# ParthaEth/GIF

Hardware: AMD Instinct MI355X
Metric: G+D train-step images/sec at 256x256, batch 32/GPU (higher is better)
Workload: dtype f32

## Files before the change

gif_amd/csrc/conv_igemm.hip:

```cpp
#include <stdlib.h>

#include <atomic>
#include <type_traits>

#include "conv_common.h"
#include "conv_route.h"

namespace {

using gif::f32x16, gif::f32x4, gif::xcd_remap;
using gif::buf_rsrc_t, gif::make_buf_rsrc, gif::buf_load_lds16;

struct GatherParams {
    const void* x;
    const void* wp;
    void* y;
    const float* in_scale;
    const float* out_scale;
    const float* bias;
    const void* residual;
    int B, Hi, Wi, Ci;
    int Ho, Wo, Co;
    int Hp, Wp;
    int os, ooy, oox;
// ... 822 lines not shown
#pragma unroll
        for (int j = 0; j < NT; ++j) bv[slot][j] = *reinterpret_cast<const frag_t*>(Bb + j * 32 * LD + c);
        if (SCALE) {
#pragma unroll
            for (int i = 0; i < MT; ++i)
                av[slot][i] *= *reinterpret_cast<const frag_t*>(Stab + s_row[i] + (pair ? (kk * 2 * EPC) & (BK / 2 - 1) : kc + kk * 2 * EPC));
        }
    };
    auto mfma_group = [&](int slot) __attribute__((always_inline)) {
        if constexpr (F16) {
#pragma unroll
            for (int i = 0; i < MT; ++i)
#pragma unroll
                for (int j = 0; j < NT; ++j)
                    acc[i][j] = __builtin_amdgcn_mfma_f32_32x32x16_f16(av[slot][i], bv[slot][j], acc[i][j], 0, 0, 0);
            __builtin_amdgcn_sched_group_barrier(0x100, MT + NT + (SCALE ? MT : 0), 0);
            __builtin_amdgcn_sched_group_barrier(0x008, MT * NT, 0);
        } else {
#pragma unroll
            for (int t = 0; t < 4; ++t)
#pragma unroll
                for (int i = 0; i < MT; ++i)
#pragma unroll
                    for (int j = 0; j < NT; ++j)
                        acc[i][j] = __builtin_amdgcn_mfma_f32_32x32x2f32(av[slot][i][t], bv[slot][j][t], acc[i][j], 0, 0, 0);
            __builtin_amdgcn_sched_group_barrier(0x100, MT + NT + (SCALE ? MT : 0), 0);
            __builtin_amdgcn_sched_group_barrier(0x008, 4 * MT * NT, 0);
        }
    };

    issue(0);
    __syncthreads();
    frag_read(0, 0, 0, 0);
    for (int step = 0; step + 1 < nsteps; ++step) {
        issue(cur ^ 1);
#pragma unroll
        for (int g = 0; g + 1 < KG; ++g) {
            frag_read(cur, g + 1, (g + 1) & 1, cmp_kc);
            mfma_group(g & 1);
        }
        __syncthreads();
        cmp_kc = next_kc(cmp_kc);
        cur ^= 1;
        frag_read(cur, 0, KG & 1, cmp_kc);
        mfma_group((KG - 1) & 1);
        if (KG & 1) {
#pragma unroll
            for (int i = 0; i < MT; ++i) av[0][i] = av[1][i];
#pragma unroll
            for (int j = 0; j < NT; ++j) bv[0][j] = bv[1][j];
        }
    }
#pragma unroll
    for (int g = 0; g < KG; ++g) {
        if (g + 1 < KG) frag_read(cur, g + 1, (g + 1) & 1, cmp_kc);
        mfma_group(g & 1);
    }
    }
    conv_epilogue<BM, BN, 32, MT, NT, T, THREADS>(p, acc, smem, m0, n0, wm0, wn0, tid, li, lh, HWp);
}

template <typename T, int BM, int BN, int WAVES_M, int WAVES_N, bool SCALE, int BK, int X3 = 0, int NST = 2>
__global__ void __launch_bounds__(64 * WAVES_M * WAVES_N, (X3 == 2 && WAVES_M * WAVES_N == 4) ? 2 : 1) conv_gather_mfma_glds(const GatherParams p) {
    glds_body<T, BM, BN, WAVES_M, WAVES_N, SCALE, BK, X3, NST>(p, (int)blockIdx.x, (int)gridDim.x);
}

struct MultiParams {
    GatherParams ph[4];
    int wg_end[4];
    int nph;
};

template <typename T, int BM, int BN, int WAVES_M, int WAVES_N, bool SCALE, int BK, int X3 = 0, int NST = 2>
__global__ void __launch_bounds__(64 * WAVES_M * WAVES_N, (X3 == 2 && WAVES_M * WAVES_N == 4) ? 2 : 1) conv_gather_mfma_glds_multi(const MultiParams mp) {
    const int b = (int)blockIdx.x;
    int k = 0;
    while (k + 1 < mp.nph && b >= mp.wg_end[k]) ++k;
    const int begin = k ? mp.wg_end[k - 1] : 0;
    glds_body<T, BM, BN, WAVES_M, WAVES_N, SCALE, BK, X3, NST>(mp.ph[k], b - begin, mp.wg_end[k] - begin);
}

constexpr int kRowsThinA = 288;

__global__ void __launch_bounds__(256, 2) conv3x3_rows_thin_h2(const GatherParams p) {
    constexpr int BM = 256, BN = 32, LD = 32, THREADS = 256, MT = 2, NT = 1, AROWS = kRowsThinA, A_IT = AROWS / 32;
    extern __shared__ __attribute__((aligned(16))) float smem[];
    float* const As = smem;
    typedef __attribute__((address_space(3))) void* lptr_t;
    const float* const px = static_cast<const float*>(p.x);
    const unsigned short* const pw = static_cast<const unsigned short*>(p.wp);

    const int tid = threadIdx.x, lane = tid & 63;
    const int wave = __builtin_amdgcn_readfirstlane(tid >> 6);
    const int li = lane & 31, lh = lane >> 5;
    const int wm0 = wave * 64;
    const int tile = xcd_remap((int)blockIdx.x, (int)gridDim.x);
    const int m0 = tile * BM;
    const int HWp = p.Hp * p.Wp;
    const int segw = p.Wp >= BM ? BM : p.Wp, seg = segw + 2, nseg = BM / segw;

    unsigned a_voff[A_IT], a_mask[A_IT];
#pragma unroll
    for (int it = 0; it < A_IT; ++it) {
        const int r = (tid >> 3) + 32 * it;
        const int sg = r / seg, j = r - sg * seg;
        const int ms = m0 + sg * segw;
        const bool in_tile = sg < nseg && ms < p.M;
        const int mm = in_tile ? ms : 0;
        const int b = mm / HWp, rr = mm - b * HWp;
        const int oy = rr / p.Wp, ox0 = rr - oy * p.Wp;
        const int ix = ox0 + j - 1;
        const bool okx = in_tile && (unsigned)ix < (unsigned)p.Wi;
        const int c4 = ((tid & 7) ^ ((r >> 1) & 7)) * 4;
        a_voff[it] = (unsigned)(((b * p.Hi + oy) * p.Wi + ix) * p.Ci + c4) * 4u;
        unsigned mk = 0;
#pragma unroll
        for (int d = 0; d < 3; ++d) mk |= ((okx && (unsigned)(oy + d - 1) < (unsigned)p.Hi) ? 1u : 0u) << d;
        a_mask[it] = mk;
    }
    const buf_rsrc_t rs_a = make_buf_rsrc(px - (size_t)p.Wi * p.Ci, 0xFFFFFFFFu);

    const int kch = p.CP / 32, nst = 3 * kch;
    auto issue_a = [&](int buf, int st) __attribute__((always_inline)) {
        const int ta = st / kch, kc = (st - ta * kch) * 32;
        const int dy = p.dy0 + ta * p.ddy;
        const int so = ((dy + 1) * p.Wi * p.Ci + kc) * 4;
        float* Ad = As + buf * AROWS * LD + wave * 8 * LD;
#pragma unroll
        for (int it = 0; it < A_IT; ++it) {
            const int r = (tid >> 3) + 32 * it;
            const int c4 = ((tid & 7) ^ ((r >> 1) & 7)) * 4;
            const unsigned bad = (__builtin_amdgcn_ubfe(a_mask[it], (unsigned)(dy + 1), 1u) - 1u) | ((kc + c4 < p.Ci) ? 0u : 0xFFFFFFFFu);
            buf_load_lds16(rs_a, (lptr_t)(Ad + it * 32 * LD), a_voff[it] | bad, so);
        }
    };
    gif::u32x4_t sb[2][3][2][2];
    auto issue_b = [&](auto set_tag, int st) __attribute__((always_inline)) {
        constexpr int set = decltype(set_tag)::value;
        const int ta = st / kch, kc = (st - ta * kch) * 32;
#pragma unroll
        for (int tb = 0; tb < 3; ++tb) {
            const int widx = (p.ky0 + ta * p.kstep) * p.KW + p.kx0 + tb * p.kstep;
#pragma unroll
            for (int q = 0; q < 2; ++q)
#pragma unroll
                for (int t = 0; t < 2; ++t)
                    sb[set][tb][q][t] = *reinterpret_cast<const gif::u32x4_t*>(pw + ((size_t)(widx * 2 + t) * p.RP + li) * p.CP + kc + q * 16 + lh * 8);
        }
    };

    f32x16 acc[MT][NT];
#pragma unroll
    for (int i = 0; i < MT; ++i)
#pragma unroll
        for (int r = 0; r < 16; ++r) acc[i][0][r] = 0.f;
    gif::H2Row hr[MT];
    int a_row[MT];
#pragma unroll
    for (int i = 0; i < MT; ++i) a_row[i] = wm0 + i * 32 + li + 2 * ((wm0 + i * 32) / segw);

    auto compute = [&](int buf, auto set_tag) __attribute__((always_inline)) {
        constexpr int set = decltype(set_tag)::value;
        const float* Ab = As + buf * AROWS * LD;
#pragma unroll
        for (int tb = 0; tb < 3; ++tb) {
            const int shift = p.dx0 + tb * p.ddx + 1;
#pragma unroll
            for (int q = 0; q < 2; ++q) {
                f32x4 ra[MT][2];
#pragma unroll
                for (int i = 0; i < MT; ++i) {
                    const int brow = a_row[i] + shift;
                    const int f = (brow >> 1) & 7;
#pragma unroll
                    for (int u = 0; u < 2; ++u) ra[i][u] = *reinterpret_cast<const f32x4*>(Ab + brow * LD + (((q * 4 + lh * 2 + u) ^ f) << 2));
                }
                gif::u32x4_t sa[2][MT];
                bool need = false;
#pragma unroll
                for (int i = 0; i < MT; ++i) gif::h2_observe(hr[i], gif::h2_group_max(ra[i][0], ra[i][1]), need);
                if (need) {
#pragma unroll
                    for (int i = 0; i < MT; ++i)
                        gif::h2_for_rows(lh, hr[i].dl, [&](int r, int d) __attribute__((always_inline)) { acc[i][0][r] = ldexpf(acc[i][0][r], d); });
                }
#pragma unroll
                for (int i = 0; i < MT; ++i)
#pragma unroll
                    for (int e = 0; e < 4; ++e) {
                        unsigned h, l;
                        gif::split_pair_h2(ra[i][e / 2][(e % 2) * 2], ra[i][e / 2][(e % 2) * 2 + 1], hr[i].sc, h, l);
                        sa[0][i][e] = h; sa[1][i][e] = l;
                    }
#pragma unroll
                for (int t3 = 0; t3 < 3; ++t3) {
                    const gif::X3Terms tm = gif::x3_terms<true>(t3);
#pragma unroll
                    for (int i = 0; i < MT; ++i)
                        acc[i][0] = __builtin_amdgcn_mfma_f32_32x32x16_f16(__builtin_bit_cast(gif::f16x8_t, sa[tm.a][i]),
                                                                           __builtin_bit_cast(gif::f16x8_t, sb[set][tb][q][tm.b]), acc[i][0], 0, 0, 0);
                }
            }
        }
    };

    issue_a(0, 0);
    issue_b(std::integral_constant<int, 0>{}, 0);
    __builtin_amdgcn_s_waitcnt(0x0F70);
    __syncthreads();
    for (int st = 0; st < nst; st += 2) {
        if (st + 1 < nst) {
            issue_a(1, st + 1);
            issue_b(std::integral_constant<int, 1>{}, st + 1);
        }
        compute(0, std::integral_constant<int, 0>{});
        __builtin_amdgcn_s_waitcnt(0x0F70);
        __syncthreads();
        if (st + 1 < nst) {
            if (st + 2 < nst) {
                issue_a(0, st + 2);
                issue_b(std::integral_constant<int, 0>{}, st + 2);
            }
            compute(1, std::integral_constant<int, 1>{});
            __builtin_amdgcn_s_waitcnt(0x0F70);
            __syncthreads();
        }
    }

    {
        bool wide = false;
#pragma unroll
        for (int i = 0; i < MT; ++i) wide |= gif::h2_wide(hr[i]);
        if (p.gate) {
            const bool wflag = p.wexp[p.RP + li] != 0;
            if (__builtin_amdgcn_ballot_w64(wide) != 0 && __builtin_amdgcn_ballot_w64(wflag) != 0 && lane == 0) atomicMax(p.gate, p.gate_gen);
        }
        const int wex = p.wexp[li];
#pragma unroll
        for (int i = 0; i < MT; ++i)
            gif::h2_for_rows(lh, hr[i].ex, [&](int r, int er) __attribute__((always_inline)) { acc[i][0][r] = ldexpf(acc[i][0][r], -(er + wex)); });
    }
    conv_epilogue<BM, BN, LD, MT, NT, float, THREADS, false, 2 * AROWS * LD>(p, acc, smem, m0, 0, wm0, 0, tid, li, lh, HWp);
}

template <int BN, int CP>
constexpr int halo_lds_floats() { return CP == 32 ? 5376 : 10496; }

template <int BN, int CP>
__global__ void __launch_bounds__(256, 3) conv_halo_f16(const GatherParams p) {
    typedef gif::f16 T;
    constexpr int TH = 16, TW = 16, BM = TH * TW;
    constexpr int CPP = CP / 8;
    constexpr int CPP_SHIFT = CPP == 4 ? 2 : 3;
    constexpr int PPS_SHIFT = CPP == 4 ? 2 : 1;
    constexpr int SWM = CPP - 1;
    constexpr int KG = CP / 16, MT = 2, NT = BN / 32;
    constexpr int HALO_HALFS = halo_lds_floats<BN, CP>() * 2;
    static_assert((CP == 32 || CP == 64) && (BN == 32 || BN == 64), "halo kernel configurations");
    extern __shared__ __attribute__((aligned(16))) float smem[];
    T* const Xs = reinterpret_cast<T*>(smem);
    T* const Wsm = Xs + HALO_HALFS;
    const T* const px = static_cast<const T*>(p.x);
    const T* const pw = static_cast<const T*>(p.wp);
    const T* const pzero = static_cast<const T*>(p.zero);
    typedef const __attribute__((address_space(1))) void* gptr_t;
    typedef __attribute__((address_space(3))) void* lptr_t;

    const int tid = threadIdx.x, lane = tid & 63;
    const int wave = __builtin_amdgcn_readfirstlane(tid >> 6);
    const int li = lane & 31, lh = lane >> 5;
    const int tile = xcd_remap((int)blockIdx.x, (int)gridDim.x);
    const int tpi = p.t2_tx * p.t2_ty;
    const int b = tile / tpi, tr = tile - b * tpi;
    const int tyi = tr / p.t2_tx, txi = tr - tyi * p.t2_tx;
    const int dy_min = p.ddy > 0 ? p.dy0 : p.dy0 + (p.nky - 1) * p.ddy;
    const int dx_min = p.ddx > 0 ? p.dx0 : p.dx0 + (p.nkx - 1) * p.ddx;
    const int HWh = TW + p.nkx - 1;
    const int nchunks = (TH + p.nky - 1) * HWh * CPP;
    const bool has_scale = p.in_scale != nullptr;

    {
        constexpr int QSTEP = 256 / CPP;
        const int dqy = QSTEP / HWh, dqx = QSTEP - dqy * HWh;
        int q = (wave * 64 + lane) >> CPP_SHIFT;
        int hy = q / HWh, hx = q - hy * HWh;
        const int cphys = lane & SWM;
        const T* const xb = px + (size_t)b * p.Hi * p.Wi * p.Ci;
        const int gy0 = tyi * TH + dy_min, gx0 = txi * TW + dx_min;
        for (int e0 = wave * 64; e0 < nchunks; e0 += 256) {
            const int c = cphys ^ ((q >> PPS_SHIFT) & SWM);
            const int gy = gy0 + hy, gx = gx0 + hx;
            const bool ok = e0 + lane < nchunks && (unsigned)gy < (unsigned)p.Hi && (unsigned)gx < (unsigned)p.Wi && c * 8 < p.Ci;
            const T* g = ok ? xb + ((gy * p.Wi + gx) * p.Ci + c * 8) : pzero;
            __builtin_amdgcn_global_load_lds((gptr_t)g, (lptr_t)(Xs + e0 * 8), 16, 0, 0);
            q += QSTEP;
            hx += dqx; hy += dqy;
            if (hx >= HWh) { hx -= HWh; ++hy; }
        }
    }
    {
        constexpr int WPT = BN * CPP;
        const int cphys = lane & SWM;
        if constexpr (WPT >= 256) {
            const int n = (wave * 64 + lane) >> CPP_SHIFT;
            const int c = cphys ^ ((n >> PPS_SHIFT) & SWM);
            int ta = 0, tb = 0;
            for (int t = 0; t < p.ntaps; ++t) {
                const int widx = (p.ky0 + ta * p.kstep) * p.KW + p.kx0 + tb * p.kstep;
                if (++tb == p.nkx) { tb = 0; ++ta; }
                const T* const wt = pw + (size_t)widx * p.RP * CP;
#pragma unroll
                for (int k = 0; k < WPT / 256; ++k)
                    __builtin_amdgcn_global_load_lds((gptr_t)(wt + (n + k * (256 / CPP)) * CP + c * 8),
                                                     (lptr_t)(Wsm + (t * WPT + k * 256 + wave * 64) * 8), 16, 0, 0);
            }
        } else {
            const int n = ((wave & 1) * 64 + lane) >> CPP_SHIFT;
            const int c = cphys ^ ((n >> PPS_SHIFT) & SWM);
            for (int t = wave >> 1; t < p.ntaps; t += 2) {
                const int a = t / p.nkx, bb = t - a * p.nkx;
                const int widx = (p.ky0 + a * p.kstep) * p.KW + p.kx0 + bb * p.kstep;
                __builtin_amdgcn_global_load_lds((gptr_t)(pw + ((size_t)widx * p.RP + n) * CP + c * 8),
                                                 (lptr_t)(Wsm + (t * WPT + (wave & 1) * 64) * 8), 16, 0, 0);
// ... 1 lines not shown
        }
    }
    gif::f16x8_t sreg[KG];
    if (has_scale) {
#pragma unroll
        for (int kg = 0; kg < KG; ++kg) {
            const int ci = kg * 16 + lh * 8;
            float4 s0 = make_float4(0.f, 0.f, 0.f, 0.f), s1 = s0;
            if (ci < p.Ci) {
                s0 = *reinterpret_cast<const float4*>(p.in_scale + (size_t)b * p.Ci + ci);
                s1 = *reinterpret_cast<const float4*>(p.in_scale + (size_t)b * p.Ci + ci + 4);
            }
            sreg[kg][0] = (T)s0.x; sreg[kg][1] = (T)s0.y; sreg[kg][2] = (T)s0.z; sreg[kg][3] = (T)s0.w;
            sreg[kg][4] = (T)s1.x; sreg[kg][5] = (T)s1.y; sreg[kg][6] = (T)s1.z; sreg[kg][7] = (T)s1.w;
        }
    }
    int boff[NT][KG], ckg[KG], q0[MT];
#pragma unroll
    for (int kg = 0; kg < KG; ++kg) {
        ckg[kg] = (kg * 2 + lh) << 4;
#pragma unroll
        for (int j = 0; j < NT; ++j) {
            const int r = j * 32 + li;
            boff[j][kg] = ((r << CPP_SHIFT) + ((kg * 2 + lh) ^ ((r >> PPS_SHIFT) & SWM))) << 4;
        }
    }
#pragma unroll
    for (int i = 0; i < MT; ++i) q0[i] = (4 * wave + 2 * i + (li >> 4)) * HWh + (li & 15);
    f32x16 acc[MT][NT];
#pragma unroll
    for (int i = 0; i < MT; ++i)
#pragma unroll
        for (int j = 0; j < NT; ++j)
#pragma unroll
            for (int r = 0; r < 16; ++r) acc[i][j][r] = 0.f;

    const char* const Xb = reinterpret_cast<const char*>(Xs);
    const char* Wb = reinterpret_cast<const char*>(Wsm);
    __syncthreads();
    int ta = 0, tb = 0;
    for (int t = 0; t < p.ntaps; ++t) {
        const int off = (p.dy0 + ta * p.ddy - dy_min) * HWh + (p.dx0 + tb * p.ddx - dx_min);
        if (++tb == p.nkx) { tb = 0; ++ta; }
        gif::f16x8_t av[KG][MT], bw[KG][NT];
#pragma unroll
        for (int j = 0; j < NT; ++j)
#pragma unroll
            for (int kg = 0; kg < KG; ++kg) bw[kg][j] = *reinterpret_cast<const gif::f16x8_t*>(Wb + boff[j][kg]);
        Wb += BN * CP * 2;
#pragma unroll
        for (int i = 0; i < MT; ++i) {
            const int q = q0[i] + off;
            const int g16 = (q << (CPP_SHIFT + 4)) ^ ((q << (4 - PPS_SHIFT)) & (SWM << 4));
#pragma unroll
            for (int kg = 0; kg < KG; ++kg) av[kg][i] = *reinterpret_cast<const gif::f16x8_t*>(Xb + (g16 ^ ckg[kg]));
        }
        if (has_scale) {
#pragma unroll
            for (int kg = 0; kg < KG; ++kg)
#pragma unroll
                for (int j = 0; j < NT; ++j) bw[kg][j] *= sreg[kg];
        }
#pragma unroll
        for (int kg = 0; kg < KG; ++kg)
#pragma unroll
            for (int i = 0; i < MT; ++i)
#pragma unroll
                for (int j = 0; j < NT; ++j)
                    acc[i][j] = __builtin_amdgcn_mfma_f32_32x32x16_f16(av[kg][i], bw[kg][j], acc[i][j], 0, 0, 0);
    }
    conv_epilogue<BM, BN, 8, MT, NT, T, 256, true, halo_lds_floats<BN, CP>()>(p, acc, smem, tile * BM, 0, wave * 64, 0, tid, li, lh, 0, b, tyi * TH, txi * TW);
}

namespace route = gif_conv;

static_assert(kRowsThinA == route::ROWS_THIN_A, "conv_route.h sizes the LDS of conv3x3_rows_thin_h2");

const route::ConvKnobs& conv_knobs() {
    static const route::ConvKnobs once = [] {
        route::ConvKnobs k;
        const auto num = gif::knob_int;
        k.h2_ring3 = num("GIF_H2_RING", 3) != 2;
        k.h2_rows_thin = num("GIF_H2_ROWS_THIN", 1) != 0;
        k.x3_waves = num("GIF_X3_WAVES", k.x3_waves);
        k.f16_tile256 = num("GIF_F16_TILE256", 1) != 0;
        k.x3_big = num("GIF_X3_BIG", 1) != 0;
        k.dense128 = num("GIF_DENSE_TILE", 128) != 256;
        k.x3_multi_big = num("GIF_X3_MULTI_BIG", 1) != 0;
        k.conv_variant = num("GIF_CONV_VARIANT", 0);
        k.f16_halo = num("GIF_F16_HALO", 1) != 0;
        return k;
    }();
    return once;
}

inline std::atomic<int>& halo_switch() {
    static std::atomic<int> on{conv_knobs().f16_halo ? 1 : 0};
    return on;
}

void fill_phase(GatherParams& p, const route::ConvPhase& q) {
    p.B = q.B; p.Hi = q.Hi; p.Wi = q.Wi; p.Ci = q.Ci;
    p.Ho = q.Ho; p.Wo = q.Wo; p.Co = q.Co;
    p.Hp = q.Hp; p.Wp = q.Wp; p.os = q.os; p.ooy = q.ooy; p.oox = q.oox; p.is = q.is;
    p.ntaps = q.ntaps; p.nky = q.nky; p.nkx = q.nkx; p.dy0 = q.dy0; p.ddy = q.ddy; p.dx0 = q.dx0; p.ddx = q.ddx;
    p.ky0 = q.ky0; p.kx0 = q.kx0; p.kstep = q.kstep; p.KW = q.KW;
    p.RP = q.RP; p.CP = q.CP; p.M = q.M; p.m_begin = 0;
    p.x3 = q.x3; p.dense = q.dense; p.pair = q.pair; p.no_split = q.no_split;
}
GatherParams launch_params(const GatherParams& phase, const route::ConvLaunch& l, int i, const void* zero) {
    GatherParams p = phase;
    if (l.kernel != route::CONV_GLDS_MULTI) { p.m_begin = l.m_begin; p.M = l.M; }
    p.tiles_m = l.tiles_m[i]; p.tiles_n = l.tiles_n;
    p.stab_nb = l.stab_nb[i]; p.stab_stride = l.stab_stride;
    p.t2_tx = l.t2_tx; p.t2_ty = l.t2_ty;
    p.part_row0 = l.part_row0[i];
    p.zero = zero;
    return p;
}

template <typename K, typename P>
void launch_kernel(K kern, gif::LdsAttr& attr, const route::ConvLaunch& l, const P& p, hipStream_t s) {
    gif::launch_lds(kern, attr, dim3((unsigned)l.grid), dim3(l.threads), l.lds_bytes, s, p);
}

template <int BM, int BN, int BK, int WMv, int WNv>
bool simple_try(const route::ConvLaunch& l, const GatherParams& p, hipStream_t s) {
    if (l.BM != BM || l.BN != BN || l.BK != BK) return false;
    static gif::LdsAttr attr;
    launch_kernel(conv_gather_mfma<BM, BN, BK, WMv, WNv>, attr, l, p, s);
    return true;
}

template <typename T, int BM, int BN, int WMv, int WNv, bool SCALE, int X3, int NST>
void glds_run(const route::ConvLaunch& l, const GatherParams& p, hipStream_t s) {
    static gif::LdsAttr attr;
    launch_kernel(conv_gather_mfma_glds<T, BM, BN, WMv, WNv, SCALE, 128 / sizeof(T), X3, NST>, attr, l, p, s);
}
template <typename T, int BM, int BN, int WMv, int WNv, int X3, int NST = 2>
bool glds_try(const route::ConvLaunch& l, const GatherParams& p, hipStream_t s) {
    if (l.X3 != X3 || l.NST != NST) return false;
    l.SCALE ? glds_run<T, BM, BN, WMv, WNv, true, X3, NST>(l, p, s) : glds_run<T, BM, BN, WMv, WNv, false, X3, NST>(l, p, s);
    return true;
}
template <typename T, int BM, int BN, int WMv, int WNv>
bool glds_tile(const route::ConvLaunch& l, const GatherParams& p, hipStream_t s) {
    if (l.f16 != (sizeof(T) == 2) || l.BM != BM || l.BN != BN || l.WM != WMv || l.WN != WNv) return false;
    if constexpr (sizeof(T) == 4) {
        if constexpr (WNv == 1 || (BM == 64 && BN == 64)) {
            if constexpr (WMv * WNv == 8)
                if (glds_try<T, BM, BN, WMv, WNv, 2, 3>(l, p, s)) return true;
            if (glds_try<T, BM, BN, WMv, WNv, 2>(l, p, s)) return true;
        }
        if (glds_try<T, BM, BN, WMv, WNv, 1>(l, p, s)) return true;
    }
    return glds_try<T, BM, BN, WMv, WNv, 0>(l, p, s);
}

template <typename T, int BM, int BN, int WMv, int WNv, bool SCALE, int X3, int NST>
void multi_run(const route::ConvLaunch& l, const MultiParams& mp, hipStream_t s) {
    static gif::LdsAttr attr;
    launch_kernel(conv_gather_mfma_glds_multi<T, BM, BN, WMv, WNv, SCALE, 128 / sizeof(T), X3, NST>, attr, l, mp, s);
}
template <typename T, int BM, int BN, int WMv, int WNv, int X3, int NST = 2>
bool multi_try(const route::ConvLaunch& l, const MultiParams& mp, hipStream_t s) {
    if (l.f16 != (sizeof(T) == 2) || l.BM != BM || l.BN != BN || l.WM != WMv || l.WN != WNv || l.X3 != X3 || l.NST != NST) return false;
    l.SCALE ? multi_run<T, BM, BN, WMv, WNv, true, X3, NST>(l, mp, s) : multi_run<T, BM, BN, WMv, WNv, false, X3, NST>(l, mp, s);
    return true;
}

template <int BN, int CP>
bool halo_try(const route::ConvLaunch& l, const GatherParams& p, hipStream_t s) {
    static_assert(halo_lds_floats<BN, CP>() == route::halo_lds_floats(CP), "conv_route.h sizes the LDS of conv_halo_f16");
    if (l.BN != BN || l.HCP != CP) return false;
    static gif::LdsAttr attr;
    launch_kernel(conv_halo_f16<BN, CP>, attr, l, p, s);
    return true;
}

int conv_dispatch(const route::ConvLaunch& l, const GatherParams* ph, hipStream_t s, const char* who) {
    using gif::f16;
    const void* zero = nullptr;
    if (l.kernel != route::CONV_SIMPLE) {
        zero = gif::zero_page16();
        GIF_REQUIRE(zero, "%s: zero page lookup failed", who);
    }
    bool launched = false;
    if (l.kernel == route::CONV_GLDS_MULTI) {
        MultiParams mp{};
        int total = 0;
        for (int i = 0; i < l.nph; ++i) {
            mp.ph[i] = launch_params(ph[l.phase0 + i], l, i, zero);
            total += l.tiles_m[i] * l.tiles_n;
            mp.wg_end[i] = total;
        }
        mp.nph = l.nph;
        launched = multi_try<float, 64, 64, 2, 2, 0>(l, mp, s) || multi_try<float, 64, 64, 2, 2, 1>(l, mp, s) ||
                   multi_try<float, 64, 64, 2, 2, 2>(l, mp, s) || multi_try<float, 256, 128, 8, 1, 1>(l, mp, s) ||
                   multi_try<float, 256, 128, 8, 1, 2>(l, mp, s) || multi_try<float, 256, 128, 8, 1, 2, 3>(l, mp, s) ||
                   multi_try<f16, 64, 64, 2, 2, 0>(l, mp, s);
    } else {
        GatherParams p = launch_params(ph[l.phase0], l, 0, zero);
        switch (l.kernel) {
        case route::CONV_SIMPLE:
            launched = simple_try<128, 128, 32, 2, 2>(l, p, s) || simple_try<128, 128, 8, 2, 2>(l, p, s) ||
                       simple_try<256, 32, 32, 4, 1>(l, p, s) || simple_try<256, 32, 8, 4, 1>(l, p, s);
            break;
        case route::CONV_GLDS:
            launched = glds_tile<float, 128, 128, 2, 2>(l, p, s) || glds_tile<float, 128, 128, 4, 1>(l, p, s) ||
                       glds_tile<float, 256, 128, 8, 1>(l, p, s) || glds_tile<float, 256, 128, 4, 2>(l, p, s) ||
                       glds_tile<float, 128, 64, 4, 1>(l, p, s) || glds_tile<float, 64, 64, 2, 2>(l, p, s) ||
                       glds_tile<float, 256, 32, 4, 1>(l, p, s) ||
                       glds_tile<f16, 256, 256, 2, 4>(l, p, s) || glds_tile<f16, 128, 128, 2, 2>(l, p, s) ||
                       glds_tile<f16, 128, 64, 2, 2>(l, p, s) || glds_tile<f16, 64, 64, 2, 2>(l, p, s) ||
                       glds_tile<f16, 256, 32, 4, 1>(l, p, s);
            break;
        case route::CONV_ROWS_THIN: {
            static gif::LdsAttr attr;
            launch_kernel(conv3x3_rows_thin_h2, attr, l, p, s);
            launched = true;
            break;
        }
        case route::CONV_HALO:
            launched = halo_try<32, 32>(l, p, s) || halo_try<32, 64>(l, p, s) || halo_try<64, 32>(l, p, s) || halo_try<64, 64>(l, p, s);
            break;
        }
    }
    GIF_REQUIRE(launched, "%s: the route names a kernel that is not built (kind %d %s %dx%d waves %dx%d x3 %d stages %d)", who, l.kernel,
                l.f16 ? "f16" : "f32", l.BM, l.BN, l.WM, l.WN, l.X3, l.NST);
    return 0;
}

int route_error(const route::ConvRoute& r) {
    const char* fmt = r.f16 ? "f16" : "bf16x3";
    switch (r.error) {
    case route::CONV_OK: return 0;
    case route::CONV_ERR_2G: gif::set_error("conv: tensors of >= 2^31 elements are not supported (32-bit offsets)"); break;
    case route::CONV_ERR_DMA:
        gif::set_error("conv (%s): the buffer-addressed activation DMA takes < 4 GiB of input and <= 32 taps (%ld elements, %d taps)%s",
                       fmt, r.err_elems, r.err_taps, r.f16 ? "" : ": use the _f32 entry point");
        break;
    case route::CONV_ERR_X3_CIN: gif::set_error("conv (bf16x3): needs >= 24 input channels (gif_conv2d_x3_eligible)"); break;
    default: gif::set_error("conv (%s): launch configuration does not fit (rc=%d)", fmt, r.err_rc);
    }
    return GIF_ENOSUP;
}

int check_geom(const gif_conv_geom* g, const char* who) {
    GIF_REQUIRE(g, "%s: null geometry", who);
    GIF_REQUIRE(g->B >= 0 && g->Hb > 0 && g->Wb > 0 && g->Hs > 0 && g->Ws > 0, "%s: bad spatial dims", who);
    GIF_REQUIRE(g->Cb > 0 && g->Cs > 0 && g->Cb % 4 == 0 && g->Cs % 4 == 0,
                "%s: channel counts must be positive multiples of 4 (Cb=%d Cs=%d)", who, g->Cb, g->Cs);
    GIF_REQUIRE(g->KH >= 1 && g->KH <= 3 && g->KW >= 1 && g->KW <= 3, "%s: kernel %dx%d unsupported", who, g->KH, g->KW);
    GIF_REQUIRE(g->stride == 1 || g->stride == 2, "%s: stride %d unsupported", who, g->stride);
    GIF_REQUIRE(g->pad >= 0, "%s: negative pad", who);
    GIF_REQUIRE((g->Hs - 1) * g->stride + g->KH - g->pad <= g->Hb + g->pad &&
                    (g->Ws - 1) * g->stride + g->KW - g->pad <= g->Wb + g->pad,
                "%s: small grid %dx%d does not fit big grid %dx%d (k=%d s=%d p=%d)", who, g->Hs, g->Ws, g->Hb,
                g->Wb, g->KH, g->stride, g->pad);
    return 0;
}

int check_tapdense(const gif_conv_geom* g, const gif_conv_epilogue* e, int cin, bool transposed, const char* who) {
    GIF_REQUIRE(gif_conv2d_x3_tapdense_steps(cin, g->KH, g->KW) > 0, "%s: tap-dense mode needs a 3x3 kernel and 8 <= Cin < 32 (got %dx%d, %d)",
                who, g->KH, g->KW, cin);
    GIF_REQUIRE(!transposed || g->stride == 1, "%s: tap-dense mode: a strided data gradient runs tap subsets per output phase", who);
    GIF_REQUIRE(!(e && e->in_scale), "%s: tap-dense mode has no per-sample input scales", who);
    return 0;
}

int sums_begin(gif::FusedSums& sums, GatherParams& p, const gif_conv_epilogue* e, long out_rows, int Co, long hw, bool single_phase,
               const char* who) {
    if (int rc = sums.carve(e, out_rows, Co, who)) return rc;
    if (!sums.active()) return 0;
    GIF_REQUIRE(!e->dot || (e->dot_src && single_phase && hw % 256 == 0),
                "%s: the dot fusion needs dot_src, a single-phase op and a multiple of 256 output pixels per sample (got %ld)", who, hw);
    p.part_cs = sums.part_cs;
    p.part_dot = sums.part_dot;
    p.part_cap = (int)sums.cap;
    return 0;
}
int sums_finish(const gif::FusedSums& sums, int Co, int B, long hw, int rows, int tile_rows, hipStream_t s, const char* who) {
    if (!sums.active()) return 0;
    GIF_REQUIRE(rows > 0 && rows <= sums.cap, "%s: partial-sum rows %d exceed the workspace (%ld)", who, rows, sums.cap);
    GIF_REQUIRE(!sums.dot || (tile_rows > 0 && hw % tile_rows == 0 && (long)rows * tile_rows == (long)B * hw),
                "%s: dot fusion: tiles of %d rows do not partition the %d samples of %ld pixels", who, tile_rows, B, hw);
    return sums.reduce(rows, Co, B, sums.dot ? (int)(hw / tile_rows) : 0, s);
}

inline int h2_operands(GatherParams& p, int RP, const void* wp2, const void* wp_fallback, hipStream_t s) {
    p.wexp = static_cast<const int*>(wp2);
    p.wp = static_cast<const char*>(wp2) + gif::h2_header_bytes(RP);
    p.gate = nullptr; p.gate_gen = 0; p.h2_stats = nullptr;
    if (wp_fallback) {
        const gif::H2Gate gt = gif::h2_next_gate(s);
        if (gt.err) return gt.err;
        p.gate = gt.word; p.gate_gen = gt.gen;
        p.h2_stats = gif::h2_stats_words();
    }
    return 0;
}
inline void h2_to_fallback(GatherParams& p, const void* wp3) {
// ... 214 lines not shown
```

gif_amd/csrc/conv_route.h:

```cpp
#pragma once
#include <stddef.h>

namespace gif_conv {

struct ConvKnobs {
    bool h2_ring3 = true;
    bool h2_rows_thin = true;
    int x3_waves = 81;
    bool f16_tile256 = true;
    bool x3_big = true;
    bool dense128 = true;
    bool x3_multi_big = true;
    int conv_variant = 0;
    bool f16_halo = true;
};

inline int cdiv(long a, long b) { return (int)((a + b - 1) / b); }

struct TileCfg {
    int BM, BN, BK;
};

inline TileCfg pick_cfg(bool f16, int cout, int cin, bool x3 = false) {
    TileCfg c;
    c.BN = cout <= 32 ? 32 : ((f16 && cout <= 64) ? 64 : 128);
    c.BK = f16 ? 64 : ((cin < 32 && !x3) ? 8 : 32);
    c.BM = c.BN == 32 ? 256 : 128;
    return c;
}

inline void pack_dims(bool f16, int cout, int cin, bool x3, int* RP, int* CP) {
    const TileCfg c = pick_cfg(f16, cout, cin, x3);
    *RP = (cout + c.BN - 1) / c.BN * c.BN;
    *CP = (cin + c.BK - 1) / c.BK * c.BK;
    if (f16 && cin <= 32) *CP = 32;
}

inline bool x3_eligible(int cout, int cin) { return cout > 0 && cin >= 24 && cin % 4 == 0; }

constexpr size_t LDS_MAX = 160 * 1024;
constexpr int ROWS_THIN_A = 288;
constexpr int halo_lds_floats(int cp) { return cp == 32 ? 5376 : 10496; }

constexpr size_t stage_bytes(int BM, int BN, int X3, int NST) {
    return X3 ? (size_t)NST * BM * 128 + (size_t)NST * (X3 == 2 ? 2 : 3) * BN * 64 : (size_t)2 * (BM + BN) * 128;
}
constexpr size_t simple_bytes(int BM, int BN, int BK) { return (size_t)2 * (BM + BN) * (BK + 4) * sizeof(float); }

inline int stab_nb(int BM, int HWp, int B) {
    const int nb = (BM - 1) / HWp + 2;
    return nb > B ? B : nb;
}
inline int stab_stride(int CP, bool f16) { return CP + (f16 ? 8 : 4); }

struct ConvShape {
    int B, Hb, Wb, Cb, Hs, Ws, Cs, KH, KW, stride, pad;
    bool f16;
    int x3;
    bool dense;
    bool scaled;
    bool dot;
};

struct ConvPhase {
    int B, Hi, Wi, Ci;
    int Ho, Wo, Co;
    int Hp, Wp;
    int os, ooy, oox;
    int is;
    int ntaps, nky, nkx, dy0, ddy, dx0, ddx, ky0, kx0, kstep, KW;
    int RP, CP;
    int M;
    int x3, dense, pair;
    bool scaled, dot;
    int no_split;
};

struct ConvPhases {
    ConvPhase ph[4];
    int nph;
    bool need_zero;
};

inline ConvPhase phase_base(const ConvShape& s, bool transposed) {
    ConvPhase p{};
    p.B = s.B;
    if (transposed) { p.Hi = s.Hs; p.Wi = s.Ws; p.Ci = s.Cs; p.Ho = s.Hb; p.Wo = s.Wb; p.Co = s.Cb; }
    else { p.Hi = s.Hb; p.Wi = s.Wb; p.Ci = s.Cb; p.Ho = s.Hs; p.Wo = s.Ws; p.Co = s.Cs; }
    pack_dims(s.f16, p.Co, p.Ci, s.x3 != 0, &p.RP, &p.CP);
    p.pair = (s.f16 && p.CP == 32) ? 1 : 0;
    p.x3 = s.x3;
    p.dense = s.dense ? p.Ci / 4 : 0;
    p.scaled = s.scaled;
    p.dot = s.dot;
    p.no_split = s.dot ? 1 : 0;
    p.KW = s.KW;
    return p;
}

inline ConvPhases conv_phases_fwd(const ConvShape& s) {
    ConvPhases r{};
    ConvPhase p = phase_base(s, false);
    p.Hp = s.Hs; p.Wp = s.Ws; p.os = 1; p.ooy = 0; p.oox = 0; p.is = s.stride;
    p.nky = s.KH; p.nkx = s.KW; p.ntaps = s.KH * s.KW;
    p.dy0 = -s.pad; p.ddy = 1; p.dx0 = -s.pad; p.ddx = 1;
    p.ky0 = 0; p.kx0 = 0; p.kstep = 1;
    p.M = p.B * p.Hp * p.Wp;
    for (ConvPhase& q : r.ph) q = p;
    r.nph = 1;
    return r;
}

inline ConvPhases conv_phases_bwd_data(const ConvShape& s) {
    ConvPhases r{};
    const ConvPhase base = phase_base(s, true);
    for (ConvPhase& q : r.ph) q = base;
    const int st = s.stride;
    const auto pmod = [st](int a) { return ((a % st) + st) % st; };
    for (int py = 0; py < st; ++py)
        for (int px = 0; px < st; ++px) {
            ConvPhase p = base;
            p.Hp = (s.Hb - py + st - 1) / st;
            p.Wp = (s.Wb - px + st - 1) / st;
            if (p.Hp <= 0 || p.Wp <= 0) continue;
            p.os = st; p.ooy = py; p.oox = px; p.is = 1;
            p.ky0 = pmod(py + s.pad); p.kx0 = pmod(px + s.pad); p.kstep = st;
            p.nky = p.ky0 < s.KH ? (s.KH - p.ky0 + st - 1) / st : 0;
            p.nkx = p.kx0 < s.KW ? (s.KW - p.kx0 + st - 1) / st : 0;
            p.ntaps = p.nky * p.nkx;
            p.dy0 = (py + s.pad - p.ky0) / st; p.ddy = -1;
            p.dx0 = (px + s.pad - p.kx0) / st; p.ddx = -1;
            if (p.ntaps == 0) { r.need_zero = true; continue; }
            p.M = p.B * p.Hp * p.Wp;
            r.ph[r.nph++] = p;
        }
    return r;
}

inline bool rows_thin_ok(const ConvPhase& p, const ConvKnobs& k) {
    const bool unit = (p.ddy == 1 || p.ddy == -1) && (p.ddx == 1 || p.ddx == -1) && p.dy0 + p.ddy == 0 && p.dx0 + p.ddx == 0;
    return k.h2_rows_thin && p.x3 == 2 && !p.dense && !p.scaled && p.nky == 3 && p.nkx == 3 && unit && p.is == 1 && p.os == 1 && p.ooy == 0 &&
           p.oox == 0 && p.RP == 32 && p.CP % 32 == 0 && p.M % 256 == 0 && p.Hp == p.Hi && p.Wp == p.Wi &&
           p.Ho == p.Hp && p.Wo == p.Wp && (p.Wp % 256 == 0 || (p.Wp >= 32 && 256 % p.Wp == 0)) &&
           ((long)p.B * p.Hi * p.Wi + p.Wi) * p.Ci * 4 < (1L << 32);
}

inline long halo_weight_bytes(const ConvPhase& p) {
    const int bn = p.RP <= 32 ? 32 : 64, cp = p.CP <= 32 ? 32 : 64;
    return (long)p.ntaps * bn * cp * 2;
}

inline bool halo_eligible(const ConvPhase& p, bool halo_on) {
    if (!halo_on || p.is != 1 || p.RP > 64 || p.CP > 64) return false;
    if (p.nky < 1 || p.nky > 3 || p.nkx < 1 || p.nkx > 3 || (p.ddy != 1 && p.ddy != -1) || (p.ddx != 1 && p.ddx != -1)) return false;
    if (p.Hp < 16 || p.Wp < 16 || (long)p.B * cdiv(p.Hp, 16) * cdiv(p.Wp, 16) >= (1L << 23)) return false;
    if (p.dot && (p.Hp % 16 || p.Wp % 16)) return false;
    if (halo_weight_bytes(p) > 36864) return false;
    return true;
}
inline bool halo_eligible_fwd(int cin, int cout, int KH, int KW, int stride, int Hs, int Ws, bool halo_on) {
    if (cin <= 0 || cout <= 0 || KH < 1 || KW < 1 || stride < 1 || Hs <= 0 || Ws <= 0) return false;
    ConvPhase p{};
    pack_dims(true, cout, cin, false, &p.RP, &p.CP);
    p.is = stride; p.nky = KH; p.nkx = KW; p.ntaps = KH * KW; p.ddy = 1; p.ddx = 1; p.Hp = Hs; p.Wp = Ws; p.B = 1;
    return halo_eligible(p, halo_on);
}

inline bool fits_32bit(const ConvPhase& p) {
    return (long)p.B * p.Hi * p.Wi * p.Ci < (1L << 31) && (long)p.B * p.Ho * p.Wo * p.Co < (1L << 31);
}
inline long tiles128(const ConvPhase& p) { return (long)cdiv(p.M, 128) * (p.RP / 128); }
inline long tiles256(const ConvPhase& p) { return (long)cdiv(p.M, 256) * (p.RP / 128); }
inline bool small_tiles(const ConvPhase& p) { return tiles128(p) < 384; }
inline bool big_tiles(const ConvPhase& p) { return tiles256(p) >= 512; }

enum ConvKernel {
    CONV_SIMPLE = 0,
    CONV_GLDS = 1,
    CONV_GLDS_MULTI = 2,
    CONV_ROWS_THIN = 3,
    CONV_HALO = 4,
};

struct ConvLaunch {
    int kernel;
    bool f16;
    int BM, BN, BK, WM, WN;
    bool SCALE;
    int X3, NST;
    int HCP;
    int m_begin, M;
    int phase0, nph;
    int tiles_m[4], tiles_n;
    long grid;
    int threads;
    size_t lds_bytes;
    int stab_nb[4], stab_stride;
    int t2_tx, t2_ty;
    int part_row0[4];
};

enum ConvError {
    CONV_OK = 0,
    CONV_ERR_2G = 1,
    CONV_ERR_DMA = 2,
    CONV_ERR_X3_CIN = 3,
    CONV_ERR_NOFIT = 4,
};

struct ConvRoute {
    ConvLaunch launch[8];
    int nlaunch;
    int part_rows;
    int tile_rows;
    bool merged;
    bool f16;
    int family;
    int error;
    long err_elems;
    int err_taps, err_rc;
};

inline int conv_family(const ConvPhase& p, bool f16) {
    return f16 ? 6 : p.dense ? (p.x3 == 2 ? 17 : 12) : p.x3 == 2 ? 13 : p.x3 ? 8 : (p.Ci >= 32 ? 0 : 5);
}

inline void push(ConvRoute& r, ConvLaunch l) {
    for (int i = 0; i < l.nph; ++i) {
        l.part_row0[i] = r.part_rows;
        r.part_rows += l.tiles_m[i];
    }
    r.tile_rows = l.BM;
    r.launch[r.nlaunch++] = l;
}

inline ConvLaunch glds_launch(const ConvPhase* ph, int phase0, int nph, bool f16, int BM, int BN, int WM, int WN, int NST, int m_begin, int M) {
    ConvLaunch l{};
    const ConvPhase& p0 = ph[phase0];
    l.kernel = nph > 1 ? CONV_GLDS_MULTI : CONV_GLDS;
    l.f16 = f16;
    l.BM = BM; l.BN = BN; l.BK = f16 ? 64 : 32; l.WM = WM; l.WN = WN;
    l.SCALE = p0.scaled;
    l.X3 = f16 ? 0 : p0.x3;
    l.NST = NST;
    l.m_begin = m_begin; l.M = M;
    l.phase0 = phase0; l.nph = nph;
    l.tiles_n = p0.RP / BN;
    l.threads = 64 * WM * WN;
    l.stab_stride = l.SCALE ? stab_stride(p0.CP, f16) : 0;
    for (int i = 0; i < nph; ++i) {
        const ConvPhase& p = ph[phase0 + i];
        l.tiles_m[i] = cdiv((nph > 1 ? p.M : M) - m_begin, BM);
        l.grid += (long)l.tiles_m[i] * l.tiles_n;
        size_t lds = stage_bytes(BM, BN, l.X3, NST);
        if (l.SCALE) {
            l.stab_nb[i] = stab_nb(BM, p.Hp * p.Wp, p.B);
            lds += (size_t)l.stab_nb[i] * l.stab_stride * (f16 ? 2 : 4);
        }
        if (lds > l.lds_bytes) l.lds_bytes = lds;
    }
    return l;
}

inline bool try_glds(ConvRoute& r, const ConvPhase* ph, int i, bool f16, const ConvKnobs& k, int BM, int BN, int WM, int WN, int m_begin, int M) {
    for (int nst = (!f16 && ph[i].x3 == 2 && WM * WN == 8 && k.h2_ring3) ? 3 : 2; nst >= 2; --nst) {
        const ConvLaunch l = glds_launch(ph, i, 1, f16, BM, BN, WM, WN, nst, m_begin, M);
        if (l.lds_bytes > LDS_MAX) continue;
        push(r, l);
        return true;
    }
    return false;
}

inline bool try_multi(ConvRoute& r, const ConvPhase* ph, int nph, bool f16, int BM, int BN, int WM, int WN, int NST) {
    const ConvLaunch l = glds_launch(ph, 0, nph, f16, BM, BN, WM, WN, NST, 0, 0);
    if (l.lds_bytes > LDS_MAX) return false;
    push(r, l);
    r.merged = true;
    return true;
}

inline void push_simple(ConvRoute& r, const ConvPhase& p, int i, int BM, int BN, int BK, int WM, int WN) {
    ConvLaunch l{};
    l.kernel = CONV_SIMPLE;
    l.BM = BM; l.BN = BN; l.BK = BK; l.WM = WM; l.WN = WN; l.NST = 2;
    l.M = p.M;
    l.phase0 = i; l.nph = 1;
    l.tiles_m[0] = cdiv(p.M, BM);
    l.tiles_n = p.RP / BN;
    l.grid = (long)l.tiles_m[0] * l.tiles_n;
    l.threads = 256;
    l.lds_bytes = simple_bytes(BM, BN, BK);
    push(r, l);
}

inline void push_rows_thin(ConvRoute& r, const ConvPhase& p, int i) {
    ConvLaunch l{};
    l.kernel = CONV_ROWS_THIN;
    l.BM = 256; l.BN = 32; l.BK = 32; l.WM = 4; l.WN = 1; l.X3 = 2; l.NST = 2;
    l.M = p.M;
    l.phase0 = i; l.nph = 1;
    l.tiles_m[0] = p.M / 256;
    l.tiles_n = 1;
    l.grid = l.tiles_m[0];
    l.threads = 256;
    l.lds_bytes = (size_t)2 * ROWS_THIN_A * 32 * sizeof(float);
    push(r, l);
}
inline void push_halo(ConvRoute& r, const ConvPhase& p, int i) {
    ConvLaunch l{};
    l.kernel = CONV_HALO;
    l.f16 = true;
    l.BM = 256; l.BN = p.RP <= 32 ? 32 : 64; l.HCP = p.CP <= 32 ? 32 : 64; l.BK = 64; l.WM = 4; l.WN = 1; l.NST = 1;
    l.M = p.M;
    l.phase0 = i; l.nph = 1;
    l.t2_tx = cdiv(p.Wp, 16);
    l.t2_ty = cdiv(p.Hp, 16);
    l.tiles_m[0] = p.B * l.t2_tx * l.t2_ty;
    l.tiles_n = 1;
    l.grid = l.tiles_m[0];
    l.threads = 256;
    l.lds_bytes = (size_t)halo_lds_floats(l.HCP) * sizeof(float) + (size_t)p.ntaps * l.BN * l.HCP * 2;
    push(r, l);
}

inline bool try_bulk_rem(ConvRoute& r, const ConvPhase* ph, int i, bool f16, const ConvKnobs& k, int BM, int WM, int WN, long slots, bool may_split) {
    const ConvPhase& p = ph[i];
    const long tn = p.RP / 128, tiles = (long)cdiv(p.M, BM) * tn, full = tiles / slots, rem = tiles % slots;
    const bool split = may_split && !p.no_split && full >= 1 && rem > 0 && rem * 2 <= slots && slots % tn == 0;
    const int m_bulk = split ? (int)(full * slots / tn) * BM : p.M;
    if (!try_glds(r, ph, i, f16, k, BM, 128, WM, WN, 0, m_bulk)) return false;
    if (split && !try_glds(r, ph, i, f16, k, 64, 64, 2, 2, m_bulk, p.M)) { r.error = CONV_ERR_NOFIT; r.err_rc = -100; }
    return true;
}

inline void route_phase(ConvRoute& r, const ConvPhase* ph, int i, bool f16, const ConvKnobs& k, bool halo_on) {
    const ConvPhase& p = ph[i];
    if (p.M <= 0 || p.ntaps <= 0) return;
    if (!fits_32bit(p)) { r.error = CONV_ERR_2G; return; }
    const long in_elems = (long)p.B * p.Hi * p.Wi * p.Ci;
    if ((p.x3 || f16) && (in_elems * (f16 ? 2 : 4) > (1L << 32) - (1L << 26) || p.nky * p.nkx > 32)) {
        r.error = CONV_ERR_DMA; r.err_elems = in_elems; r.err_taps = p.nky * p.nkx;
        return;
    }
    const TileCfg c = pick_cfg(f16, p.Co, p.Ci, p.x3 != 0);
    const bool only_glds = f16 || p.x3;
    const bool glds = only_glds || (c.BK == 32 && k.conv_variant != 1);
    if (p.x3 && p.Ci < 24 && !p.dense) { r.error = CONV_ERR_X3_CIN; return; }
    const auto whole = [&](int BM, int BN, int WM, int WN) { return try_glds(r, ph, i, f16, k, BM, BN, WM, WN, 0, p.M); };
    const auto nofit = [&] { r.error = CONV_ERR_NOFIT; r.err_rc = -100; };
    if (f16) {
        if (halo_eligible(p, halo_on)) return push_halo(r, p, i);
        if (c.BN == 64) {
            if (!whole(128, 64, 2, 2)) nofit();
            return;
        }
        if (k.f16_tile256 && c.BN == 128 && p.RP % 256 == 0 && (long)cdiv(p.M, 256) * (p.RP / 256) >= 512 && whole(256, 256, 2, 4)) return;
    }
    if (c.BN == 128 && (f16 || c.BK == 32)) {
        if (p.x3 && small_tiles(p) && (long)cdiv(p.M, 128) * (p.RP / 64) >= 256 && whole(128, 64, 4, 1)) return;
        if (glds && small_tiles(p) && whole(64, 64, 2, 2)) return;
        if (p.x3 && k.x3_big && big_tiles(p) && !(p.dense && k.dense128)) {
            const bool w42 = k.x3_waves == 42 && p.x3 == 1;
            if (try_bulk_rem(r, ph, i, f16, k, 256, w42 ? 4 : 8, w42 ? 2 : 1, 256, true)) return;
        }
        if (glds) {
            const bool w41 = p.x3 == 2 || (p.x3 && k.x3_waves != 42);
            if (try_bulk_rem(r, ph, i, f16, k, 128, w41 ? 4 : 2, w41 ? 1 : 2, 512, k.conv_variant != 3)) return;
            if (only_glds) return nofit();
        }
        return push_simple(r, p, i, 128, 128, 32, 2, 2);
    }
    if (rows_thin_ok(p, k)) return push_rows_thin(r, p, i);
    if (only_glds) {
        if (!whole(256, 32, 4, 1)) nofit();
        return;
    }
    if (c.BN == 128) return push_simple(r, p, i, 128, 128, 8, 2, 2);
    if (c.BK == 32) {
        if (glds && whole(256, 32, 4, 1)) return;
        return push_simple(r, p, i, 256, 32, 32, 4, 1);
    }
    push_simple(r, p, i, 256, 32, 8, 4, 1);
}

inline ConvRoute conv_route(const ConvPhase* ph, int nph, bool f16, const ConvKnobs& k, bool halo_on) {
    ConvRoute r{};
    r.f16 = f16;
    r.family = conv_family(ph[0], f16);
    if (nph > 1 && k.conv_variant == 0) {
        const TileCfg c = pick_cfg(f16, ph[0].Co, ph[0].Ci, ph[0].x3 != 0);
        const bool wide = c.BN == 128 && (f16 || c.BK == 32);
        bool small_all = wide, big_all = wide && ph[0].x3 && k.x3_multi_big;
        for (int i = 0; i < nph; ++i) {
            small_all = small_all && small_tiles(ph[i]) && fits_32bit(ph[i]);
            big_all = big_all && big_tiles(ph[i]) && fits_32bit(ph[i]);
        }
        if (small_all) try_multi(r, ph, nph, f16, 64, 64, 2, 2, 2);
        else if (big_all) try_multi(r, ph, nph, f16, 256, 128, 8, 1, (ph[0].x3 == 2 && k.h2_ring3) ? 3 : 2);
    }
    if (!r.merged)
        for (int i = 0; i < nph && !r.error; ++i) route_phase(r, ph, i, f16, k, halo_on);
    return r;
}

}
```

Baseline: 180.5.

## Fold horizontal 3x3 taps into per-tap accumulators in rows-thin conv kernel

Adds a FOLD variant of the rows-thin 3x3 conv kernel that reads only the centre-shifted A rows once per K chunk and accumulates each horizontal tap into its own accumulator. After the main loop it shifts the two outer tap results through LDS and sums them, with masking at segment edges. The aim is to reuse one A fragment and one hi/lo split for all three horizontal taps instead of reloading and resplitting per shift. In exchange it triples the accumulator registers, adds an LDS pass and a sync in the epilogue, and changes the B prefetch schedule. It is gated by a new knob, on by default, for Wp dividing 256 and CP>=64.

```diff
diff --git a/gif_amd/csrc/conv_igemm.hip b/gif_amd/csrc/conv_igemm.hip
--- a/gif_amd/csrc/conv_igemm.hip
+++ b/gif_amd/csrc/conv_igemm.hip
@@ -928,6 +928,7 @@
 
 constexpr int kRowsThinA = 288;
 
+template <bool FOLD>
 __global__ void __launch_bounds__(256, 2) conv3x3_rows_thin_h2(const GatherParams p) {
     constexpr int BM = 256, BN = 32, LD = 32, THREADS = 256, MT = 2, NT = 1, AROWS = kRowsThinA, A_IT = AROWS / 32;
     extern __shared__ __attribute__((aligned(16))) float smem[];
@@ -967,7 +968,7 @@
     const buf_rsrc_t rs_a = make_buf_rsrc(px - (size_t)p.Wi * p.Ci, 0xFFFFFFFFu);
 
     const int kch = p.CP / 32, nst = 3 * kch;
-    auto issue_a = [&](int buf, int st) __attribute__((always_inline)) {
+    auto issue_a = [&](int buf, int st, unsigned dead = 0u) __attribute__((always_inline)) {
         const int ta = st / kch, kc = (st - ta * kch) * 32;
         const int dy = p.dy0 + ta * p.ddy;
         const int so = ((dy + 1) * p.Wi * p.Ci + kc) * 4;
@@ -977,9 +978,16 @@
             const int r = (tid >> 3) + 32 * it;
             const int c4 = ((tid & 7) ^ ((r >> 1) & 7)) * 4;
             const unsigned bad = (__builtin_amdgcn_ubfe(a_mask[it], (unsigned)(dy + 1), 1u) - 1u) | ((kc + c4 < p.Ci) ? 0u : 0xFFFFFFFFu);
-            buf_load_lds16(rs_a, (lptr_t)(Ad + it * 32 * LD), a_voff[it] | bad, so);
+            buf_load_lds16(rs_a, (lptr_t)(Ad + it * 32 * LD), a_voff[it] | bad | dead, so);
         }
     };
+    f32x16 acc[MT][NT];
+    gif::H2Row hr[MT];
+    int a_row[MT];
+#pragma unroll
+    for (int i = 0; i < MT; ++i) a_row[i] = wm0 + i * 32 + li + 2 * ((wm0 + i * 32) / segw);
+
+    if constexpr (!FOLD) {
     gif::u32x4_t sb[2][3][2][2];
     auto issue_b = [&](auto set_tag, int st) __attribute__((always_inline)) {
         constexpr int set = decltype(set_tag)::value;
@@ -995,15 +1003,10 @@
         }
     };
 
-    f32x16 acc[MT][NT];
 #pragma unroll
     for (int i = 0; i < MT; ++i)
 #pragma unroll
         for (int r = 0; r < 16; ++r) acc[i][0][r] = 0.f;
-    gif::H2Row hr[MT];
-    int a_row[MT];
-#pragma unroll
-    for (int i = 0; i < MT; ++i) a_row[i] = wm0 + i * 32 + li + 2 * ((wm0 + i * 32) / segw);
 
     auto compute = [&](int buf, auto set_tag) __attribute__((always_inline)) {
         constexpr int set = decltype(set_tag)::value;
@@ -1085,6 +1088,132 @@
 #pragma unroll
         for (int i = 0; i < MT; ++i)
             gif::h2_for_rows(lh, hr[i].ex, [&](int r, int er) __attribute__((always_inline)) { acc[i][0][r] = ldexpf(acc[i][0][r], -(er + wex)); });
+    }
+    } else {
+    gif::u32x4_t sb[2][3][2];
+    auto issue_b = [&](auto q_tag, int st) __attribute__((always_inline)) {
+        constexpr int q = decltype(q_tag)::value;
+        const int ta = st / kch, kc = (st - ta * kch) * 32;
+#pragma unroll
+        for (int tb = 0; tb < 3; ++tb) {
+            const int widx = (p.ky0 + ta * p.kstep) * p.KW + p.kx0 + tb * p.kstep;
+#pragma unroll
+            for (int t = 0; t < 2; ++t)
+                sb[q][tb][t] = *reinterpret_cast<const gif::u32x4_t*>(pw + ((size_t)(widx * 2 + t) * p.RP + li) * p.CP + kc + q * 16 + lh * 8);
+        }
+    };
+
+    f32x16 tacc[MT][3];
+#pragma unroll
+    for (int i = 0; i < MT; ++i)
+#pragma unroll
+        for (int tb = 0; tb < 3; ++tb)
+#pragma unroll
+            for (int r = 0; r < 16; ++r) tacc[i][tb][r] = 0.f;
+
+    auto compute = [&](int buf, auto q_tag) __attribute__((always_inline)) {
+        constexpr int q = decltype(q_tag)::value;
+        const float* Ab = As + buf * AROWS * LD;
+        f32x4 ra[MT][2];
+#pragma unroll
+        for (int i = 0; i < MT; ++i) {
+            const int brow = a_row[i] + 1;
+            const int f = (brow >> 1) & 7;
+#pragma unroll
+            for (int u = 0; u < 2; ++u) ra[i][u] = *reinterpret_cast<const f32x4*>(Ab + brow * LD + (((q * 4 + lh * 2 + u) ^ f) << 2));
+        }
+        gif::u32x4_t sa[2][MT];
+        bool need = false;
+#pragma unroll
+        for (int i = 0; i < MT; ++i) gif::h2_observe(hr[i], gif::h2_group_max(ra[i][0], ra[i][1]), need);
+        if (need) {
+#pragma unroll
+            for (int i = 0; i < MT; ++i)
+                gif::h2_for_rows(lh, hr[i].dl, [&](int r, int d) __attribute__((always_inline)) {
+#pragma unroll
+                    for (int tb = 0; tb < 3; ++tb) tacc[i][tb][r] = ldexpf(tacc[i][tb][r], d);
+                });
+        }
+#pragma unroll
+        for (int i = 0; i < MT; ++i)
+#pragma unroll
+            for (int e = 0; e < 4; ++e) {
+                unsigned h, l;
+                gif::split_pair_h2(ra[i][e / 2][(e % 2) * 2], ra[i][e / 2][(e % 2) * 2 + 1], hr[i].sc, h, l);
+                sa[0][i][e] = h; sa[1][i][e] = l;
+            }
+#pragma unroll
+        for (int t3 = 0; t3 < 3; ++t3) {
+            const gif::X3Terms tm = gif::x3_terms<true>(t3);
+#pragma unroll
+            for (int tb = 0; tb < 3; ++tb)
+#pragma unroll
+                for (int i = 0; i < MT; ++i)
+                    tacc[i][tb] = __builtin_amdgcn_mfma_f32_32x32x16_f16(__builtin_bit_cast(gif::f16x8_t, sa[tm.a][i]),
+                                                                         __builtin_bit_cast(gif::f16x8_t, sb[q][tb][tm.b]), tacc[i][tb], 0, 0, 0);
+        }
+    };
+    auto stage = [&](int buf, int st) __attribute__((always_inline)) {
+        const bool more = st + 1 < nst;
+        issue_b(std::integral_constant<int, 1>{}, st);
+        issue_a(buf ^ 1, more ? st + 1 : st, more ? 0u : 0xFFFFFFFFu);
+        compute(buf, std::integral_constant<int, 0>{});
+        issue_b(std::integral_constant<int, 0>{}, more ? st + 1 : st);
+        compute(buf, std::integral_constant<int, 1>{});
+        __builtin_amdgcn_s_waitcnt(0x0F70);
+        __syncthreads();
+    };
+
+    issue_a(0, 0);
+    issue_b(std::integral_constant<int, 0>{}, 0);
+    __builtin_amdgcn_s_waitcnt(0x0F70);
+    __syncthreads();
+    for (int st = 0; st < nst; st += 2) {
+        stage(0, st);
+        if (st + 1 < nst) stage(1, st + 1);
+    }
+
+    {
+        bool wide = false;
+#pragma unroll
+        for (int i = 0; i < MT; ++i) wide |= gif::h2_wide(hr[i]);
+        if (p.gate) {
+            const bool wflag = p.wexp[p.RP + li] != 0;
+            if (__builtin_amdgcn_ballot_w64(wide) != 0 && __builtin_amdgcn_ballot_w64(wflag) != 0 && lane == 0) atomicMax(p.gate, p.gate_gen);
+        }
+        const int wex = p.wexp[li];
+#pragma unroll
+        for (int i = 0; i < MT; ++i)
+            gif::h2_for_rows(lh, hr[i].ex, [&](int r, int er) __attribute__((always_inline)) {
+#pragma unroll
+                for (int tb = 0; tb < 3; ++tb) tacc[i][tb][r] = ldexpf(tacc[i][tb][r], -(er + wex));
+            });
+    }
+    {
+        static_assert(2 * BM * 32 <= 2 * AROWS * LD, "the two outer taps' planes fit the staging buffers");
+        float* const Ts = smem;
+#pragma unroll
+        for (int i = 0; i < MT; ++i)
+#pragma unroll
+            for (int r = 0; r < 16; ++r) {
+                const int row = wm0 + i * 32 + gif::acc_row(r, lh);
+                Ts[row * 32 + li] = tacc[i][0][r];
+                Ts[(BM + row) * 32 + li] = tacc[i][2][r];
+            }
+        __syncthreads();
+        const int dxa = p.dx0, dxc = p.dx0 + 2 * p.ddx;
+#pragma unroll
+        for (int i = 0; i < MT; ++i)
+#pragma unroll
+            for (int r = 0; r < 16; ++r) {
+                const int row = wm0 + i * 32 + gif::acc_row(r, lh);
+                const int col = row & (segw - 1);
+                const bool oka = (unsigned)(col + dxa) < (unsigned)segw, okc = (unsigned)(col + dxc) < (unsigned)segw;
+                const float ta = Ts[(oka ? row + dxa : row) * 32 + li];
+                const float tc = Ts[(BM + (okc ? row + dxc : row)) * 32 + li];
+                acc[i][0][r] = ((oka ? ta : 0.f) + tacc[i][1][r]) + (okc ? tc : 0.f);
+            }
+    }
     }
     conv_epilogue<BM, BN, LD, MT, NT, float, THREADS, false, 2 * AROWS * LD>(p, acc, smem, m0, 0, wm0, 0, tid, li, lh, HWp);
 }
@@ -1252,6 +1381,7 @@
         const auto num = gif::knob_int;
         k.h2_ring3 = num("GIF_H2_RING", 3) != 2;
         k.h2_rows_thin = num("GIF_H2_ROWS_THIN", 1) != 0;
+        k.h2_rows_fold = num("GIF_H2_ROWS_FOLD", 1) != 0;
         k.x3_waves = num("GIF_X3_WAVES", k.x3_waves);
         k.f16_tile256 = num("GIF_F16_TILE256", 1) != 0;
         k.x3_big = num("GIF_X3_BIG", 1) != 0;
@@ -1386,8 +1516,9 @@
                        glds_tile<f16, 256, 32, 4, 1>(l, p, s);
             break;
         case route::CONV_ROWS_THIN: {
-            static gif::LdsAttr attr;
-            launch_kernel(conv3x3_rows_thin_h2, attr, l, p, s);
+            static gif::LdsAttr attr, attr_fold;
+            if (l.fold) launch_kernel(conv3x3_rows_thin_h2<true>, attr_fold, l, p, s);
+            else launch_kernel(conv3x3_rows_thin_h2<false>, attr, l, p, s);
             launched = true;
             break;
         }
diff --git a/gif_amd/csrc/conv_route.h b/gif_amd/csrc/conv_route.h
--- a/gif_amd/csrc/conv_route.h
+++ b/gif_amd/csrc/conv_route.h
@@ -13,6 +13,7 @@
     bool x3_multi_big = true;
     int conv_variant = 0;
     bool f16_halo = true;
+    bool h2_rows_fold = true;
 };
 
 inline int cdiv(long a, long b) { return (int)((a + b - 1) / b); }
@@ -145,6 +146,8 @@
            ((long)p.B * p.Hi * p.Wi + p.Wi) * p.Ci * 4 < (1L << 32);
 }
 
+inline bool rows_fold_ok(const ConvPhase& p, const ConvKnobs& k) { return k.h2_rows_fold && p.Wp <= 256 && 256 % p.Wp == 0 && p.CP >= 64; }
+
 inline long halo_weight_bytes(const ConvPhase& p) {
     const int bn = p.RP <= 32 ? 32 : 64, cp = p.CP <= 32 ? 32 : 64;
     return (long)p.ntaps * bn * cp * 2;
@@ -198,6 +201,7 @@
     int stab_nb[4], stab_stride;
     int t2_tx, t2_ty;
     int part_row0[4];
+    bool fold;
 };
 
 enum ConvError {
@@ -294,7 +298,7 @@
     push(r, l);
 }
 
-inline void push_rows_thin(ConvRoute& r, const ConvPhase& p, int i) {
+inline void push_rows_thin(ConvRoute& r, const ConvPhase& p, int i, const ConvKnobs& k) {
     ConvLaunch l{};
     l.kernel = CONV_ROWS_THIN;
     l.BM = 256; l.BN = 32; l.BK = 32; l.WM = 4; l.WN = 1; l.X3 = 2; l.NST = 2;
@@ -305,6 +309,7 @@
     l.grid = l.tiles_m[0];
     l.threads = 256;
     l.lds_bytes = (size_t)2 * ROWS_THIN_A * 32 * sizeof(float);
+    l.fold = rows_fold_ok(p, k);
     push(r, l);
 }
 inline void push_halo(ConvRoute& r, const ConvPhase& p, int i) {
@@ -371,7 +376,7 @@
         }
         return push_simple(r, p, i, 128, 128, 32, 2, 2);
     }
-    if (rows_thin_ok(p, k)) return push_rows_thin(r, p, i);
+    if (rows_thin_ok(p, k)) return push_rows_thin(r, p, i, k);
     if (only_glds) {
         if (!whole(256, 32, 4, 1)) nofit();
         return;
```

Result: no change. 180.9, median of 5 (+0.3%).
